# JiahaoPlus/EvoWorld

Measured on AMD Instinct MI355X. Metric: panoramic frames/sec per clip (576x1024x25f, 25 denoise steps), higher is better.
Workload: dtype f16

## Files before the change

evoworld_amd/csrc/norm.hip:

```cpp
#include "common.h"
#include <cstdlib>

namespace {

inline int gn_chunks(int n_slabs, int rows) {
    constexpr int target = 640;
    int want = (target + n_slabs - 1) / n_slabs;
    const int cap = (rows + 63) / 64;
    if (want > cap) want = cap;
    if (want > 512) want = 512;
    return want < 1 ? 1 : want;
}

__device__ __forceinline__ void gn_chan(float& na, float& ma, float& Ma, float nb, float mb, float Mb) {
    if (nb > 0.f) {
        const float n = na + nb, w = __fdividef(nb, n), d = mb - ma;
        ma = fmaf(d, w, ma);
        Ma = fmaf(d * d, na * w, Ma + Mb);
        na = n;
    }
}

__global__ void gn_stats_kernel(const f16* __restrict__ x, const int8_t* __restrict__ x_lo, float* __restrict__ part,
                                int rows, int C_src, int c_off, int C_tot, int VPP, int PL, int rows_per_block) {
    extern __shared__ float lds[];
    const int tid = threadIdx.x;
    const int slab = blockIdx.y;
    const int v = tid % VPP, pl = tid / VPP;
    const int r0 = blockIdx.x * rows_per_block;
    const int r1 = min(rows, r0 + rows_per_block);
    const int nb = max(r1 - r0, 0), nlo = nb / PL, nrem = nb - nlo * PL;
    const int nt = nlo + (pl < nrem ? 1 : 0);
    float s[8], q[8], piv[8];
    const size_t slab_off = ((size_t)slab * rows) * C_src + v * 8;
    const f16* base = x + slab_off;
    const int8_t* base_lo = x_lo ? x_lo + slab_off : nullptr;
#pragma unroll
    for (int e = 0; e < 8; ++e) { s[e] = 0.f; q[e] = 0.f; piv[e] = 0.f; }
    if (nt > 0) {
        const size_t o = (size_t)(r0 + pl) * C_src;
        const f16x8 p0 = *(const f16x8*)(base + o);
#pragma unroll
        for (int e = 0; e < 8; ++e) piv[e] = (float)p0[e];
        if (base_lo) ew_split_dec8(p0, *(const u32x2*)(base_lo + o), piv);
    }
    int r = r0 + pl;
    if (base_lo) {
        constexpr int UL = 8;
        for (; r + (UL - 1) * PL < r1; r += UL * PL) {
            f16x8 val[UL];
            u32x2 vlo[UL];
#pragma unroll
            for (int u = 0; u < UL; ++u) {
                val[u] = *(const f16x8*)(base + (size_t)(r + u * PL) * C_src);
                vlo[u] = *(const u32x2*)(base_lo + (size_t)(r + u * PL) * C_src);
            }
#pragma unroll
            for (int u = 0; u < UL; ++u) {
                float xv[8];
                ew_split_dec8(val[u], vlo[u], xv);
#pragma unroll
                for (int e = 0; e < 8; ++e) {
                    const float f = xv[e] - piv[e];
                    s[e] += f;
                    q[e] += f * f;
                }
            }
        }
        for (; r < r1; r += PL) {
            const f16x8 val = *(const f16x8*)(base + (size_t)r * C_src);
            float xv[8];
            ew_split_dec8(val, *(const u32x2*)(base_lo + (size_t)r * C_src), xv);
#pragma unroll
            for (int e = 0; e < 8; ++e) {
                const float f = xv[e] - piv[e];
                s[e] += f;
                q[e] += f * f;
            }
        }
    } else {
        for (; r + 7 * PL < r1; r += 8 * PL) {
            f16x8 val[8];
#pragma unroll
            for (int u = 0; u < 8; ++u) val[u] = *(const f16x8*)(base + (size_t)(r + u * PL) * C_src);
#pragma unroll
            for (int u = 0; u < 8; ++u)
#pragma unroll
                for (int e = 0; e < 8; ++e) {
                    const float f = (float)val[u][e] - piv[e];
                    s[e] += f;
                    q[e] += f * f;
                }
        }
        for (; r < r1; r += PL) {
            const f16x8 val = *(const f16x8*)(base + (size_t)r * C_src);
#pragma unroll
            for (int e = 0; e < 8; ++e) {
                const float f = (float)val[e] - piv[e];
                s[e] += f;
                q[e] += f * f;
            }
        }
    }
    float* mine = lds + (size_t)pl * 2 * C_src;
    const float inv_n = 1.f / (float)max(nt, 1);
#pragma unroll
    for (int e = 0; e < 8; ++e) {
        const float d = s[e] * inv_n;
        mine[v * 8 + e] = piv[e] + d;
        mine[C_src + v * 8 + e] = fmaxf(q[e] - s[e] * d, 0.f);
    }
    __syncthreads();
    float* dst = part + (((size_t)slab * gridDim.x + blockIdx.x) * C_tot + c_off) * 2;
    for (int c = tid; c < C_src; c += blockDim.x) {
        const float ref = lds[c];
        float sd = 0.f;
        for (int k = 0; k < PL; ++k) sd += (float)(nlo + (k < nrem ? 1 : 0)) * (lds[(size_t)k * 2 * C_src + c] - ref);
        const float dm = nb > 0 ? sd / (float)nb : 0.f;
        float M2 = 0.f;
        for (int k = 0; k < PL; ++k) {
            const float dk = lds[(size_t)k * 2 * C_src + c] - ref - dm;
            M2 += lds[(size_t)k * 2 * C_src + C_src + c] + (float)(nlo + (k < nrem ? 1 : 0)) * dk * dk;
        }
        *(f32x2*)(dst + 2 * c) = (f32x2){ref + dm, M2};
    }
}

__global__ __launch_bounds__(256) void gn_finalize_kernel(const float* __restrict__ part, float* __restrict__ stats, int n_slabs,
                                                          int rows, int C_tot, int groups, int chunks) {
    __shared__ float red[3][256];
    __shared__ float chan[2][512];
    __shared__ float wsum[4];
    const int tid = threadIdx.x;
    const int slab = blockIdx.x / groups, g = blockIdx.x - slab * groups;
    const int gs = C_tot / groups;
    const float n = (float)rows;
    const int cw = gs < 256 ? gs : 256;
    const int KP = 256 / cw;
    const int rpb = (rows + chunks - 1) / chunks;
    for (int c0 = 0; c0 < gs; c0 += cw) {
        const int c = c0 + tid % cw, kc = tid / cw;
        float na = 0.f, ma = 0.f, Ma = 0.f, ref = 0.f;
        if (kc < KP && c < gs) {
            const float* p = part + (((size_t)slab * chunks) * C_tot + g * gs + c) * 2;
            ref = p[0];
            for (int k = kc; k < chunks; k += KP) {
                const f32x2 v = *(const f32x2*)(p + (size_t)k * C_tot * 2);
                gn_chan(na, ma, Ma, (float)max(min(rows - k * rpb, rpb), 0), v[0] - ref, v[1]);
            }
        }
        red[0][tid] = na;
        red[1][tid] = ma;
        red[2][tid] = Ma;
        __syncthreads();
        if (tid < cw && c0 + tid < gs) {
            const int lanes = min(KP, chunks);
            float sd = 0.f, M = 0.f;
            for (int k = 0; k < lanes; ++k) sd += red[0][k * cw + tid] * red[1][k * cw + tid];
            const float dm = sd / n;
            for (int k = 0; k < lanes; ++k) {
                const float dk = red[1][k * cw + tid] - dm;
                M += red[2][k * cw + tid] + red[0][k * cw + tid] * dk * dk;
            }
            chan[0][c0 + tid] = ref + dm;
            chan[1][c0 + tid] = M;
        }
        __syncthreads();
    }
    float ms = 0.f, m2 = 0.f;
    for (int c = tid; c < gs; c += 256) { ms += chan[0][c]; m2 += chan[1][c]; }
    ms = wave_sum(ms);
    m2 = wave_sum(m2);
    if ((tid & 63) == 0) wsum[tid >> 6] = ms;
    __syncthreads();
    const float mean = (wsum[0] + wsum[1] + wsum[2] + wsum[3]) / (float)gs;
    __syncthreads();
    float dev = 0.f;
    for (int c = tid; c < gs; c += 256) { const float d = chan[0][c] - mean; dev += d * d; }
    dev = wave_sum(dev);
    if ((tid & 63) == 0) { wsum[tid >> 6] = m2 + n * dev; }
    __syncthreads();
    if (tid == 0) *(f32x2*)(stats + (size_t)blockIdx.x * 2) = (f32x2){mean, (wsum[0] + wsum[1] + wsum[2] + wsum[3]) / (n * (float)gs)};
}

template <bool LO, bool YLO>
__global__ void gn_apply_kernel(const f16* __restrict__ x, const int8_t* __restrict__ x_lo, const float* __restrict__ stats,
                                const f16* __restrict__ gamma, const f16* __restrict__ beta, f16* __restrict__ y,
                                f16* __restrict__ y_lo, int ld_y, int rows,
                                int C_src, int c_off, int C_tot, int groups, float eps, int silu, int VPP, int PL,
                                int rows_per_block) {
    const int tid = threadIdx.x;
    const int slab = blockIdx.y;
    const int v = tid % VPP, pl = tid / VPP;
    const int c = v * 8;
    const int gs = C_tot / groups;
    const f16x8 gm = *(const f16x8*)(gamma + c_off + c);
    const f16x8 bt = *(const f16x8*)(beta + c_off + c);
    float scale[8], shift[8];
    int gprev = -1;
    float mean = 0.f, rstd = 0.f;
#pragma unroll
    for (int e = 0; e < 8; ++e) {
        const int g = (c_off + c + e) / gs;
        if (g != gprev) {
            gprev = g;
            const f32x2 st = *(const f32x2*)(stats + ((size_t)slab * groups + g) * 2);
            mean = st[0];
            rstd = rsqrtf(st[1] + eps);
        }
        scale[e] = rstd;
        shift[e] = mean;
    }
    const int r0 = blockIdx.x * rows_per_block;
    const int r1 = min(rows, r0 + rows_per_block);
    const f16* xin = x + ((size_t)slab * rows) * C_src + c;
    const int8_t* xlo = LO ? x_lo + ((size_t)slab * rows) * C_src + c : nullptr;
    f16* yout = y + ((size_t)slab * rows) * ld_y + c_off + c;
    f16* ylo = YLO ? y_lo + ((size_t)slab * rows) * ld_y + c_off + c : nullptr;
    int r = r0 + pl;
    for (; r + 3 * PL < r1; r += 4 * PL) {
        f16x8 val[4];
        u32x2 vlo[4];
#pragma unroll
        for (int u = 0; u < 4; ++u) {
            val[u] = *(const f16x8*)(xin + (size_t)(r + u * PL) * C_src);
            if constexpr (LO) vlo[u] = *(const u32x2*)(xlo + (size_t)(r + u * PL) * C_src);
        }
#pragma unroll
        for (int u = 0; u < 4; ++u) {
            f16x8 o, ol;
#pragma unroll
            for (int e = 0; e < 8; ++e) {
                float xv;
                if constexpr (LO) xv = ew_split_dec(val[u][e], ew_sbyte(vlo[u][e >> 2], e & 3));
                else xv = (float)val[u][e];
                float f = (xv - shift[e]) * scale[e] * (float)gm[e] + (float)bt[e];
                if (silu) f = ew_silu(f);
                o[e] = (f16)f;
                if constexpr (YLO) ol[e] = (f16)(f - (float)o[e]);
            }
            *(f16x8*)(yout + (size_t)(r + u * PL) * ld_y) = o;
            if constexpr (YLO) *(f16x8*)(ylo + (size_t)(r + u * PL) * ld_y) = ol;
        }
    }
    for (; r < r1; r += PL) {
        const f16x8 val = *(const f16x8*)(xin + (size_t)r * C_src);
        u32x2 vlo;
        if constexpr (LO) vlo = *(const u32x2*)(xlo + (size_t)r * C_src);
        f16x8 o, ol;
#pragma unroll
        for (int e = 0; e < 8; ++e) {
            float xv;
            if constexpr (LO) xv = ew_split_dec(val[e], ew_sbyte(vlo[e >> 2], e & 3));
            else xv = (float)val[e];
            float f = (xv - shift[e]) * scale[e] * (float)gm[e] + (float)bt[e];
            if (silu) f = ew_silu(f);
            o[e] = (f16)f;
            if constexpr (YLO) ol[e] = (f16)(f - (float)o[e]);
        }
        *(f16x8*)(yout + (size_t)r * ld_y) = o;
        if constexpr (YLO) *(f16x8*)(ylo + (size_t)r * ld_y) = ol;
    }
}

template <int NV, int RPW>
__global__ __launch_bounds__(256) void ln_kernel(const f16* __restrict__ x, const int8_t* __restrict__ x_lo,
                                                 const f16* __restrict__ addvec, int rpg, f16* __restrict__ x_out,
                                                 int8_t* __restrict__ x_out_lo, const f16* __restrict__ gamma,
                                                 const f16* __restrict__ beta, f16* __restrict__ y, int rows, int C,
                                                 float eps) {
    const int lane = threadIdx.x & 63;
    const int row0 = (blockIdx.x * 4 + (threadIdx.x >> 6)) * RPW;
    if (row0 >= rows) return;
    const int VPP = C / 8;
    float v[RPW][NV][8];
    f16x8 raw[RPW][NV], add[RPW][NV];
    u32x2 rlo[RPW][NV];
#pragma unroll
    for (int r = 0; r < RPW; ++r) {
        const int row = min(row0 + r, rows - 1);
#pragma unroll
        for (int k = 0; k < NV; ++k) {
            const int vi = lane + k * 64;
            if (vi < VPP) {
                raw[r][k] = *(const f16x8*)(x + (size_t)row * C + vi * 8);
                if (x_lo) rlo[r][k] = *(const u32x2*)(x_lo + (size_t)row * C + vi * 8);
                if (addvec) add[r][k] = *(const f16x8*)(addvec + (size_t)(row / rpg) * C + vi * 8);
            }
        }
    }
    f16x8 g[NV], bta[NV];
#pragma unroll
    for (int k = 0; k < NV; ++k) {
        const int vi = lane + k * 64;
        if (vi < VPP) { g[k] = *(const f16x8*)(gamma + vi * 8); bta[k] = *(const f16x8*)(beta + vi * 8); }
    }
#pragma unroll
    for (int r = 0; r < RPW; ++r) {
        const int row = row0 + r;
        const bool live = row < rows;
        float sum = 0.f;
#pragma unroll
        for (int k = 0; k < NV; ++k) {
            const int vi = lane + k * 64;
            if (vi < VPP) {
                if (x_lo) {
                    ew_split_dec8(raw[r][k], rlo[r][k], v[r][k]);
                } else {
#pragma unroll
                    for (int e = 0; e < 8; ++e) v[r][k][e] = (float)raw[r][k][e];
                }
                if (addvec) {
                    f16x8 xo;
                    int s8[8];
#pragma unroll
                    for (int e = 0; e < 8; ++e) {
                        const float sum = v[r][k][e] + (float)add[r][k][e];
                        xo[e] = (f16)sum;
                        s8[e] = ew_split_enc(sum, xo[e]);
                        v[r][k][e] = !x_out ? sum : (x_out_lo ? ew_split_dec(xo[e], s8[e]) : (float)xo[e]);
                    }
                    if (x_out && live) *(f16x8*)(x_out + (size_t)row * C + vi * 8) = xo;
                    if (x_out_lo && live)
                        *(u32x2*)(x_out_lo + (size_t)row * C + vi * 8) =
                            (u32x2){ew_pack4(s8[0], s8[1], s8[2], s8[3]), ew_pack4(s8[4], s8[5], s8[6], s8[7])};
                }
#pragma unroll
                for (int e = 0; e < 8; ++e) sum += v[r][k][e];
            } else {
#pragma unroll
                for (int e = 0; e < 8; ++e) v[r][k][e] = 0.f;
            }
        }
        const float mean = wave_sum(sum) / (float)C;
        float sq = 0.f;
#pragma unroll
        for (int k = 0; k < NV; ++k) {
            const int vi = lane + k * 64;
            if (vi < VPP) {
#pragma unroll
                for (int e = 0; e < 8; ++e) { const float d = v[r][k][e] - mean; sq += d * d; }
            }
        }
        const float rstd = rsqrtf(wave_sum(sq) / (float)C + eps);
#pragma unroll
        for (int k = 0; k < NV; ++k) {
            const int vi = lane + k * 64;
            if (vi < VPP && live) {
                f16x8 o;
#pragma unroll
                for (int e = 0; e < 8; ++e) o[e] = (f16)((v[r][k][e] - mean) * rstd * (float)g[k][e] + (float)bta[k][e]);
                *(f16x8*)(y + (size_t)row * C + vi * 8) = o;
            }
        }
    }
}

}

extern "C" size_t ew_groupnorm_workspace_floats(int n_slabs, int rows, int C_tot, int groups) {
    if (n_slabs <= 0 || rows <= 0 || C_tot <= 0 || groups <= 0) return 0;
    return (size_t)n_slabs * gn_chunks(n_slabs, rows) * C_tot * 2 + (size_t)n_slabs * groups * 2;
}

namespace {
struct GnWs { float* part; float* stats; int chunks; };
inline GnWs gn_ws(float* ws, int n_slabs, int rows, int C_tot) {
    GnWs w;
    w.chunks = gn_chunks(n_slabs, rows);
    w.part = ws;
    w.stats = ws + (size_t)n_slabs * w.chunks * C_tot * 2;
    return w;
}
}

extern "C" ew_status ew_groupnorm_stats_f16(const void* x, const void* x_lo, float* ws, int n_slabs, int rows, int C_src,
                                            int c_off, int C_tot, int groups, void* stream) {
    EW_REQUIRE(x && ws, "ew_groupnorm_stats_f16: null pointer");
    EW_REQUIRE(n_slabs > 0 && rows > 0 && C_src > 0 && C_src % 8 == 0 && C_src <= 8192, "ew_groupnorm_stats_f16: bad shape");
    EW_REQUIRE(groups > 0 && C_tot % groups == 0 && c_off >= 0 && c_off + C_src <= C_tot, "ew_groupnorm_stats_f16: bad groups");
    const int VPP = C_src / 8;
    EW_REQUIRE(VPP <= 1024, "ew_groupnorm_stats_f16: C_src too large");
    const int PL = VPP >= 256 ? 1 : 256 / VPP;
    const GnWs w = gn_ws(ws, n_slabs, rows, C_tot);
    const int rpb = ew_cdiv(rows, w.chunks);
    dim3 grid(w.chunks, n_slabs);
    const size_t lds = (size_t)PL * 2 * C_src * sizeof(float);
    EW_REQUIRE(lds <= 64 * 1024, "ew_groupnorm_stats_f16: C_src too large for the LDS combine");
    hipLaunchKernelGGL(gn_stats_kernel, grid, dim3(VPP * PL), lds, (hipStream_t)stream, (const f16*)x, (const int8_t*)x_lo,
                       w.part, rows, C_src, c_off, C_tot, VPP, PL, rpb);
    return ew_check_launch("ew_groupnorm_stats_f16");
}

extern "C" ew_status ew_groupnorm_finalize(float* ws, int n_slabs, int rows, int C_tot, int groups, void* stream) {
    EW_REQUIRE(ws, "ew_groupnorm_finalize: null pointer");
    EW_REQUIRE(n_slabs > 0 && rows > 0 && groups > 0 && C_tot % groups == 0 && C_tot / groups <= 512,
               "ew_groupnorm_finalize: bad shape");
    const GnWs w = gn_ws(ws, n_slabs, rows, C_tot);
    hipLaunchKernelGGL(gn_finalize_kernel, dim3(n_slabs * groups), dim3(256), 0, (hipStream_t)stream,
                       w.part, w.stats, n_slabs, rows, C_tot, groups, w.chunks);
    return ew_check_launch("ew_groupnorm_finalize");
}

static ew_status gn_apply_launch(const char* what, const void* x, const void* x_lo, const float* ws, const void* gamma,
                                 const void* beta, void* y, void* y_lo, int ld_y, int n_slabs, int rows, int C_src, int c_off,
                                 int C_tot, int groups, float eps, int silu, void* stream) {
    EW_REQUIRE(x && ws && gamma && beta && y, "ew_groupnorm_apply: null pointer");
    EW_REQUIRE(n_slabs > 0 && rows > 0 && C_src > 0 && C_src % 8 == 0 && c_off % 8 == 0 && C_tot % 8 == 0,
               "ew_groupnorm_apply: bad shape");
    EW_REQUIRE(groups > 0 && C_tot % groups == 0 && c_off >= 0 && c_off + C_src <= C_tot, "ew_groupnorm_apply: bad groups");
    EW_REQUIRE(ld_y >= C_tot && ld_y % 8 == 0, "ew_groupnorm_apply: bad output row stride");
    const int VPP = C_src / 8;
    EW_REQUIRE(VPP <= 1024, "ew_groupnorm_apply: C_src too large");
    const int PL = VPP >= 256 ? 1 : 256 / VPP;
    const int rpb = 8 * PL;
    const GnWs w = gn_ws((float*)ws, n_slabs, rows, C_tot);
    dim3 grid(ew_cdiv(rows, rpb), n_slabs);
#define GN_APPLY(LO_, YLO_)                                                                                                      \
    hipLaunchKernelGGL((gn_apply_kernel<LO_, YLO_>), grid, dim3(VPP * PL), 0, (hipStream_t)stream, (const f16*)x,                  \
                       (const int8_t*)x_lo, w.stats, (const f16*)gamma, (const f16*)beta, (f16*)y, (f16*)y_lo, ld_y, rows, C_src,  \
                       c_off, C_tot, groups, eps, silu, VPP, PL, rpb)
    if (x_lo) { if (y_lo) GN_APPLY(true, true); else GN_APPLY(true, false); }
    else      { if (y_lo) GN_APPLY(false, true); else GN_APPLY(false, false); }
#undef GN_APPLY
    return ew_check_launch(what);
}

extern "C" ew_status ew_groupnorm_apply_f16(const void* x, const void* x_lo, const float* ws, const void* gamma,
                                            const void* beta, void* y, int n_slabs, int rows, int C_src, int c_off, int C_tot,
                                            int groups, float eps, int silu, void* stream) {
    return gn_apply_launch("ew_groupnorm_apply_f16", x, x_lo, ws, gamma, beta, y, nullptr, C_tot, n_slabs, rows, C_src, c_off, C_tot,
                           groups, eps, silu, stream);
}

extern "C" ew_status ew_groupnorm_apply_split_f16(const void* x, const void* x_lo, const float* ws, const void* gamma,
                                                  const void* beta, void* y, void* y_lo, int ld_y, int n_slabs, int rows, int C_src,
                                                  int c_off, int C_tot, int groups, float eps, int silu, void* stream) {
    EW_REQUIRE(y_lo, "ew_groupnorm_apply_split_f16: null pointer");
    return gn_apply_launch("ew_groupnorm_apply_split_f16", x, x_lo, ws, gamma, beta, y, y_lo, ld_y, n_slabs, rows, C_src, c_off, C_tot,
                           groups, eps, silu, stream);
}

extern "C" ew_status ew_layernorm_f16(const void* x, const void* x_lo, const void* addvec, int rows_per_group, void* x_out,
                                      void* x_out_lo, const void* gamma, const void* beta, void* y, int rows, int C, float eps,
                                      void* stream) {
    EW_REQUIRE(x && gamma && beta && y, "ew_layernorm_f16: null pointer");
    EW_REQUIRE(rows > 0 && C > 0 && C % 8 == 0 && C <= 2048, "ew_layernorm_f16: need C %% 8 == 0 and C <= 2048 (C=%d)", C);
    EW_REQUIRE(!addvec || rows_per_group >= 1, "ew_layernorm_f16: rows_per_group must be >= 1");
    EW_REQUIRE(!x_out_lo || (addvec && x_out), "ew_layernorm_f16: x_out_lo needs addvec and x_out");
    const int nv = (C / 8 + 63) / 64;
    dim3 block(256);
    hipStream_t s = (hipStream_t)stream;
    const int rpg = rows_per_group >= 1 ? rows_per_group : 1;
#define LN_LAUNCH(NV, RPW)                                                                                         \
    hipLaunchKernelGGL((ln_kernel<NV, RPW>), dim3(ew_cdiv(rows, 4 * RPW)), block, 0, s, (const f16*)x, (const int8_t*)x_lo, \
                       (const f16*)addvec, rpg, (f16*)x_out, (int8_t*)x_out_lo, (const f16*)gamma, (const f16*)beta, (f16*)y, rows, C, eps)
    if (nv == 1) LN_LAUNCH(1, 4);
    else if (nv == 2) LN_LAUNCH(2, 4);
    else if (nv == 3) LN_LAUNCH(3, 2);
    else LN_LAUNCH(4, 2);
#undef LN_LAUNCH
    return ew_check_launch("ew_layernorm_f16");
}
```

evoworld_amd/ops.py:

```python
import ctypes

import numpy as np
import torch

from . import _lib
from ._lib import GemmArgs

A_DENSE, A_CONV3X3, A_CONVT3 = _lib.EW_A_DENSE, _lib.EW_A_CONV3X3, _lib.EW_A_CONVT3
ACT_NONE, ACT_SILU, ACT_GEGLU, ACT_GELU = _lib.EW_ACT_NONE, _lib.EW_ACT_SILU, _lib.EW_ACT_GEGLU, _lib.EW_ACT_GELU

_zero_pages = {}


def _stream():
    return ctypes.c_void_p(torch.cuda.current_stream().cuda_stream)


def _ptr(t):
    return None if t is None else ctypes.c_void_p(t.data_ptr())


def _call(name, *args):
    _lib.check(getattr(_lib.load(), name)(*args, _stream()), name)


def _aligned(t, n=16):
    t = t.contiguous()
    return t if t.data_ptr() % n == 0 else t.clone(memory_format=torch.contiguous_format)


def _req(t, dtype, name):
    if t.device.type != "cuda":
        raise _lib.EvoWorldHipError(f"{name} must live on the GPU (got {t.device}); evoworld_amd has no CPU path")
    if t.dtype != dtype:
        raise TypeError(f"{name}: expected {dtype}, got {t.dtype}")
    if not t.is_contiguous():
        raise ValueError(f"{name} must be contiguous")
    return t


def zero_page(device):
    key = str(device)
    if key not in _zero_pages:
        _zero_pages[key] = torch.zeros(4096, dtype=torch.float16, device=device)
    return _zero_pages[key]


class Res:
    __slots__ = ("hi", "lo")

    def __init__(self, hi, lo=None):
        self.hi, self.lo = hi, lo

    @classmethod
    def empty(cls, rows, C, device, split):
        hi = torch.empty(rows, C, dtype=torch.float16, device=device)
        return cls(hi, torch.empty(rows, C, dtype=torch.int8, device=device) if split else None)

    @classmethod
    def from_float(cls, x):
        x = x.float().contiguous()
        hi = x.half()
        d = (x.view(torch.int32) - hi.float().view(torch.int32) + 16) >> 5
        return cls(hi, d.clamp_(-128, 127).to(torch.int8))

    def float(self):
        if self.lo is None:
            return self.hi.float()
        return (self.hi.float().contiguous().view(torch.int32) + (self.lo.to(torch.int32) << 5)).view(torch.float32)


def _hl(x):
    if x is None:
        return None, None
    if isinstance(x, Res):
        return x.hi, x.lo
    return x, None


def gemm(a, w, out, *, M, N, c1, lda, a2=None, c2=0, lda2=0, bias=None, rowbias=None, rows_per_group=1, ld_rowbias=None,
         r1=None, ld_r1=0, r2=None, ld_r2=0, ld_out=None, mode=A_DENSE, conv=None, tconv=None, act=ACT_NONE,
         c_acc=1.0, c_r1=1.0, c_r2=1.0, conv_shift=0):
    g = GemmArgs()
    r1h, r1l = _hl(r1)
    r2h, r2l = _hl(r2)
    outh, outl = _hl(out)
    g.a, g.a2, g.w, g.bias, g.rowbias = _ptr(a), _ptr(a2), _ptr(w), _ptr(bias), _ptr(rowbias)
    g.r1, g.r2, g.out, g.zero_page = _ptr(r1h), _ptr(r2h), _ptr(outh), _ptr(zero_page(a.device))
    g.r1_lo, g.r2_lo, g.out_lo = _ptr(r1l), _ptr(r2l), _ptr(outl)
    g.M, g.N, g.c1, g.c2, g.lda, g.lda2 = M, N, c1, c2, lda, lda2
    n_out = N // 2 if act == ACT_GEGLU else N
    g.ld_out = ld_out if ld_out is not None else n_out
    g.ld_r1, g.ld_r2, g.mode = ld_r1, ld_r2, mode
    g.ld_rowbias = ld_rowbias if ld_rowbias is not None else N
    if conv is not None:
        g.n_img, g.h_in, g.w_in, g.h_out, g.w_out, g.stride, g.upsample = conv
    if tconv is not None:
        g.tB, g.tT, g.tP = tconv
    g.rows_per_group, g.act = rows_per_group, act
    g.c_acc, g.c_r1, g.c_r2 = c_acc, c_r1, c_r2
    g.conv_shift = conv_shift
    _call("ew_gemm_f16", ctypes.byref(g))
    return out


_sk_ready = set()


def streamk_init():
    key = (torch.cuda.current_device(), torch.cuda.current_stream().cuda_stream)
    if key in _sk_ready:
        return
    if _lib.load().ew_get_gemm_generation() != 3:
        return
    if torch.cuda.is_current_stream_capturing():
        return
    _sk_ready.add(key)
    if _lib.load().ew_gemm_streamk_init(_stream()) != 0:
        import warnings
        msg = _lib.load().ew_last_error()
        warnings.warn("ew_gemm_streamk_init: " + (msg.decode() if msg else "failed") + " (continuing without the stream-K tail on this stream)")


def streamk_check():
    st = _lib.load().ew_gemm_streamk_status()
    if st != 0:
        msg = _lib.load().ew_last_error()
        raise _lib.EvoWorldHipError((msg.decode() if msg else "stream-K hand-over timed out in ew_gemm_f16 (generation 3): results of that launch are invalid")
                                    if st > 0 else "ew_gemm_streamk_status: HIP error while reading the status word")


def linear(x, w, bias=None, out=None, split_out=False, **kw):
    _req(x, torch.float16, "x"); _req(w, torch.float16, "w")
    M, K = x.shape
    N = w.shape[0]
    act = kw.get("act", ACT_NONE)
    if out is None:
        n_out = N // 2 if act == ACT_GEGLU else N
        out = Res.empty(M, n_out, x.device, True) if split_out else torch.empty(M, n_out, dtype=torch.float16, device=x.device)
    return gemm(x, w, out, M=M, N=N, c1=K, lda=K, bias=bias, **kw)


class WorkspacePool:

    def __init__(self, device, floats=8 << 20):
        self.buf = torch.empty(floats, dtype=torch.float32, device=device)
        self.cur = 0

    def reset(self):
        self.cur = 0

    def take(self, n):
        n = (n + 63) // 64 * 64
        if self.cur + n > self.buf.numel():
            return torch.empty(n, dtype=torch.float32, device=self.buf.device)
        v = self.buf[self.cur: self.cur + n]
        self.cur += n
        return v


def groupnorm(xs, gamma, beta, n_slabs, rows, eps, silu, groups=32, out=None, pool=None, stats_hi_only=False, split_out=False):
    lib = _lib.load()
    srcs = [_hl(x) for x in xs]
    C_tot = sum(h.shape[-1] for h, _ in srcs)
    dev = srcs[0][0].device
    nws = lib.ew_groupnorm_workspace_floats(n_slabs, rows, C_tot, groups)
    ws = pool.take(nws) if pool is not None else torch.empty(nws, dtype=torch.float32, device=dev)
    if out is None:
        out = torch.empty(n_slabs * rows, 2 * C_tot if split_out else C_tot, dtype=torch.float16, device=dev)
    off = 0
    for h, l in srcs:
        _call("ew_groupnorm_stats_f16", _ptr(h), None if stats_hi_only else _ptr(l), _ptr(ws), n_slabs, rows, h.shape[-1], off, C_tot, groups)
        off += h.shape[-1]
    _call("ew_groupnorm_finalize", _ptr(ws), n_slabs, rows, C_tot, groups)
    off = 0
    for h, l in srcs:
        if split_out:
            _call("ew_groupnorm_apply_split_f16", _ptr(h), _ptr(l), _ptr(ws), _ptr(gamma), _ptr(beta), _ptr(out), _ptr(out[:, C_tot:]),
                  2 * C_tot, n_slabs, rows, h.shape[-1], off, C_tot, groups, eps, 1 if silu else 0)
        else:
            _call("ew_groupnorm_apply_f16", _ptr(h), _ptr(l), _ptr(ws), _ptr(gamma), _ptr(beta), _ptr(out), n_slabs, rows,
                  h.shape[-1], off, C_tot, groups, eps, 1 if silu else 0)
        off += h.shape[-1]
    return out


def layernorm(x, gamma, beta, eps=1e-5, addvec=None, rows_per_group=1, x_out=None, out=None):
    xh, xl = _hl(x)
    oh, ol = _hl(x_out)
    rows, C = xh.shape
    if out is None:
        out = torch.empty_like(xh)
    _call("ew_layernorm_f16", _ptr(xh), _ptr(xl), _ptr(addvec), rows_per_group, _ptr(oh), _ptr(ol), _ptr(gamma), _ptr(beta), _ptr(out), rows, C, eps)
    return out


def attn_spatial(q, k, vt, o, n_seq, S, heads, ld_qk, ld_vt, ld_o, scale=0.125):
    _call("ew_attn_spatial_f16", _ptr(q), _ptr(k), _ptr(vt), _ptr(o), n_seq, S, heads, ld_qk, ld_vt, ld_o, scale)
    return o


QK_LOG2_PRESCALE = (0.125 * 1.4426950408889634) ** 0.5


def attn_spatial_log2(q, k, vt, o, n_seq, S, heads, ld_qk, ld_vt, ld_o):
    _call("ew_attn_spatial_log2_f16", _ptr(q), _ptr(k), _ptr(vt), _ptr(o), n_seq, S, heads, ld_qk, ld_vt, ld_o)
    return o


def quant_rows_fp8(x):
    _req(x, torch.float16, "x")
    if x.ndim != 2:
        raise ValueError(f"x: expected fp16 [rows, K], got {tuple(x.shape)}")
    rows, K = x.shape
    q = torch.empty(rows, K, dtype=torch.uint8, device=x.device)
    scale = torch.empty(rows, dtype=torch.float32, device=x.device)
    _call("ew_quant_rows_fp8", _ptr(x), _ptr(q), _ptr(scale), rows, K)
    return q, scale


def gemm_fp8(aq, a_scale, wq, w_scale, out=None, c_acc=1.0):
    _req(aq, torch.uint8, "aq"); _req(wq, torch.uint8, "wq"); _req(a_scale, torch.float32, "a_scale"); _req(w_scale, torch.float32, "w_scale")
    if aq.ndim != 2 or wq.ndim != 2 or aq.shape[1] != wq.shape[1]:
        raise ValueError(f"aq {tuple(aq.shape)} / wq {tuple(wq.shape)}: expected [M, K] and [N, K]")
    M, K = aq.shape
    N = wq.shape[0]
    if a_scale.numel() != M or w_scale.numel() != N:
        raise ValueError(f"a_scale / w_scale hold {a_scale.numel()} / {w_scale.numel()} values for M, N = {M}, {N}")
    if out is None:
        out = torch.empty(M, N, dtype=torch.float16, device=aq.device)
    if out.dtype != torch.float16 or out.device != aq.device or tuple(out.shape) != (M, N) or out.stride(1) != 1:
        raise ValueError(f"out: expected an fp16 [{M}, {N}] device tensor with unit column stride, got {out.dtype} {tuple(out.shape)} strides {out.stride()}")
    _call("ew_gemm_fp8", _ptr(aq), _ptr(a_scale), _ptr(wq), _ptr(w_scale), _ptr(out), M, N, K, out.stride(0), float(c_acc))
    return out


def attn_temporal(q, k, v, o, B, T, S, heads, ld, ld_o, scale=0.125):
    _call("ew_attn_temporal_f16", _ptr(q), _ptr(k), _ptr(v), _ptr(o), B, T, S, heads, ld, ld_o, scale)
    return o


def softmax_rows(scores, out=None):
    h, l = _hl(scores)
    R, C = h.shape
    if out is None:
        out = torch.empty_like(h)
    _call("ew_softmax_rows_f16", _ptr(h), _ptr(l), _ptr(out), R, C, C)
    return out


def time_conv3(x, w, bias):
    _req(x, torch.float32, "x"); _req(w, torch.float32, "w"); _req(bias, torch.float32, "bias")
    B, T, C, H, W = x.shape
    y = torch.empty_like(x)
    _call("ew_time_conv3_f32", _ptr(x), _ptr(w), _ptr(bias), _ptr(y), B, T, C, H * W)
    return y


def sinusoid_embed(vals, n_rows, dim):
    _req(vals, torch.float32, "vals")
    out = torch.empty(n_rows, dim, dtype=torch.float16, device=vals.device)
    _call("ew_sinusoid_embed_f16", _ptr(vals), vals.numel(), n_rows, dim, _ptr(out))
    return out


def nchw_f32_to_nhwc_f16(x, y, ldc, c_off=0, scale=1.0, split=None):
    _req(x, torch.float32, "x"); _req(y, torch.float16, "y")
    N, C, H, W = x.shape
    if split:
        _call("ew_nchw_f32_to_nhwc_split_f16", _ptr(x), _ptr(y), N, C, H, W, ldc, c_off, split[0], split[1], scale)
        return y
    _call("ew_nchw_f32_to_nhwc_f16", _ptr(x), _ptr(y), N, C, H, W, ldc, c_off, scale)
    return y


def nhwc_f16_to_nchw_f32(x, N, C, H, W, ldc):
    _req(x, torch.float16, "x")
    y = torch.empty(N, C, H, W, dtype=torch.float32, device=x.device)
    _call("ew_nhwc_f16_to_nchw_f32", _ptr(x), _ptr(y), N, C, H, W, ldc)
    return y


def euler_cfg_step(eps, ld_eps, latents, guidance, sigma, sigma_next, next_in, cpad, T, h, w, split=None):
    _req(latents, torch.float32, "latents"); _req(guidance, torch.float32, "guidance")
    if split:
        _call("ew_euler_cfg_step_split", _ptr(eps), ld_eps, _ptr(latents), _ptr(guidance), float(sigma), float(sigma_next),
              _ptr(next_in), cpad, split[0], split[1], T, h, w)
        return
    _call("ew_euler_cfg_step", _ptr(eps), ld_eps, _ptr(latents), _ptr(guidance), float(sigma), float(sigma_next), _ptr(next_in), cpad, T, h, w)


def plucker_embed(rays, c2w):
    _req(rays, torch.float32, "rays"); _req(c2w, torch.float32, "c2w")
    H, W, _ = rays.shape
    N = c2w.shape[0]
    out = torch.empty(N, 6, H, W, dtype=torch.float32, device=rays.device)
    _call("ew_plucker_embed", _ptr(rays), _ptr(c2w), _ptr(out), N, H, W)
    return out


def cube2equi_gather(faces, lut, H, W):
    _req(faces, torch.uint8, "faces"); _req(lut, torch.int16, "lut")
    V, res, ch = faces.shape[0], faces.shape[2], faces.shape[-1]
    pano = torch.empty(V, H, W, 3, dtype=torch.uint8, device=faces.device)
    _call("ew_cube2equi_gather", _ptr(faces), ch, _ptr(lut), _ptr(pano), V, H, W, res)
    return pano


def equi2cube(panos, interpolation=True, out=None):
    _req(panos, torch.uint8, "panos")
    if panos.ndim != 4 or panos.shape[3] != 3:
        raise ValueError(f"panos: expected uint8 [V,H,W,3], got {tuple(panos.shape)}")
    V, H, W, _ = panos.shape
    if out is None:
        out = torch.empty(V, 3 * (W // 4), W, 3, dtype=torch.uint8, device=panos.device)
    _req(out, torch.uint8, "out")
    if tuple(out.shape) != (V, 3 * (W // 4), W, 3):
        raise ValueError(f"out: expected {(V, 3 * (W // 4), W, 3)}, got {tuple(out.shape)}")
    _call("ew_equi2cube_u8", _ptr(panos), _ptr(out), V, H, W, int(bool(interpolation)))
    return out


def cubemap_faces_to_equi(faces, H, W):
    from .reprojection import FACE_ORDER, build_cubemap2equi_lut
    if isinstance(faces, dict):
        unknown = set(faces) - set(FACE_ORDER)
        if unknown or not faces:
            raise ValueError(f"faces: expected keys among {FACE_ORDER}, got {sorted(faces)}")
        first = next(iter(faces.values()))
        for n, f in faces.items():
            if f.ndim != 4 or f.shape[1] != f.shape[2] or f.shape[3] != 3 or f.shape != first.shape:
                raise ValueError(f"faces[{n!r}]: expected square uint8 [V,res,res,3] faces of one size, got {tuple(f.shape)}")
        faces = torch.stack([faces[n] if n in faces else torch.zeros_like(first) for n in FACE_ORDER], dim=1)
    lut = build_cubemap2equi_lut(W, H, faces.shape[2]).to(faces.device)
    return cube2equi_gather(faces.contiguous(), lut, H, W)


def select_kth(x, k):
    lib = _lib.load()
    x = _aligned(x)
    _req(x, torch.float32, "x")
    ws = torch.empty(lib.ew_select_workspace_bytes() // 4 + 4, dtype=torch.int32, device=x.device)
    out = torch.empty(2, dtype=torch.float32, device=x.device)
    _call("ew_select_kth_f32", _ptr(x), x.numel(), int(k), _ptr(ws), _ptr(out))
    return out


def filter_compact(conf, thr, xyz, img, img_nchw_hw=0):
    lib = _lib.load()
    conf, xyz, img = _aligned(conf), _aligned(xyz), _aligned(img)
    _req(conf, torch.float32, "conf"); _req(xyz, torch.float32, "xyz"); _req(img, torch.float32, "img")
    n = conf.numel()
    dev = conf.device
    out_xyz = torch.empty(n, 3, dtype=torch.float32, device=dev)
    out_rgbx = torch.empty(n, 4, dtype=torch.uint8, device=dev)
    ws = torch.empty(lib.ew_filter_compact_workspace_bytes(n) // 4 + 1, dtype=torch.int32, device=dev)
    total = torch.zeros(1, dtype=torch.int32, device=dev)
    _call("ew_filter_compact", _ptr(conf), n, float(thr), _ptr(xyz), _ptr(img), 1 if img_nchw_hw else 0, int(img_nchw_hw),
          _ptr(out_xyz), _ptr(out_rgbx), _ptr(ws), _ptr(total))
    m = int(total.item())
    return out_xyz[:m], out_rgbx[:m]


def depth_unproject(depth, extr, intr):
    _req(depth, torch.float32, "depth"); _req(extr, torch.float32, "extr"); _req(intr, torch.float32, "intr")
    S, H, W = depth.shape
    xyz = torch.empty(S, H, W, 3, dtype=torch.float32, device=depth.device)
    _call("ew_depth_unproject", _ptr(depth), _ptr(extr), _ptr(intr), _ptr(xyz), S, H, W)
    return xyz


def splat_cubemap(xyz, rgb, w2c, res, fx, fy, cx, cy, z_near, face_channels=3):
    xyz = _aligned(xyz)
    _req(xyz, torch.float32, "xyz"); _req(w2c, torch.float32, "w2c")
    if rgb.dtype != torch.uint8 or rgb.device.type != "cuda":
        raise TypeError("rgb must be a uint8 device tensor")
    if rgb.ndim == 2 and rgb.stride(0) == 4 and rgb.stride(1) == 1:
        stride = 4
    else:
        rgb, stride = rgb.contiguous(), 3
    V = w2c.shape[0]
    zbuf = torch.empty((V, 6, res, res), dtype=torch.int64, device=xyz.device)
    _call("ew_splat_cubemap", _ptr(xyz), xyz.shape[0], _ptr(w2c), _ptr(zbuf), V, res, fx, fy, cx, cy, z_near)
    faces = torch.empty(V, 6, res, res, face_channels, dtype=torch.uint8, device=xyz.device)
    _call("ew_splat_resolve", _ptr(zbuf), _ptr(rgb), stride, _ptr(faces), face_channels, V, res)
    return faces, zbuf


def points_bounds(xyz):
    lib = _lib.load()
    xyz = _aligned(xyz)
    _req(xyz, torch.float32, "xyz")
    n = xyz.shape[0]
    if xyz.ndim != 2 or xyz.shape[1] != 3:
        raise ValueError(f"xyz must be [n,3], got {tuple(xyz.shape)}")
    ws = torch.empty(lib.ew_points_bounds_workspace_bytes(n) // 8 + 1, dtype=torch.int64, device=xyz.device)
    out6 = torch.empty(6, dtype=torch.float32, device=xyz.device)
    cnt = torch.empty(1, dtype=torch.int64, device=xyz.device)
    _call("ew_points_bounds", _ptr(xyz), n, _ptr(ws), _ptr(out6), _ptr(cnt))
    b = out6.cpu().numpy()
    return b[:3].copy(), b[3:].copy(), int(cnt.item())


VOXEL_GRID_BITS = 21


def voxel_downsample(xyz, rgbx, voxel_size):
    try:
        v = float(voxel_size)
    except (TypeError, ValueError):
        raise ValueError(f"voxel_size must be a positive finite number, got {voxel_size!r}") from None
    v32 = np.float32(v)
    if not (np.isfinite(v32) and v32 > 0):
        raise ValueError(f"voxel_size must be a positive finite number (in float32), got {voxel_size!r}")
    if rgbx.dtype != torch.uint8 or rgbx.device.type != "cuda":
        raise TypeError("rgbx must be a uint8 device tensor")
    if xyz.ndim != 2 or xyz.shape[1] != 3 or rgbx.ndim != 2 or rgbx.shape[0] != xyz.shape[0] or rgbx.shape[1] not in (3, 4):
        raise ValueError(f"xyz must be [n,3] and rgbx [n,3|4], got {tuple(xyz.shape)} and {tuple(rgbx.shape)}")
    dev = xyz.device

    def empty():
        return (torch.empty(0, 3, dtype=torch.float32, device=dev), torch.empty(0, 4, dtype=torch.uint8, device=dev),
                torch.empty(0, dtype=torch.int32, device=dev))

    n = xyz.shape[0]
    if n == 0:
        return empty()
    lib = _lib.load()
    xyz = _aligned(xyz)
    _req(xyz, torch.float32, "xyz")
    if rgbx.shape[1] == 3:
        rgbx = torch.cat([rgbx, torch.zeros(n, 1, dtype=torch.uint8, device=dev)], dim=1)
    rgbx = _aligned(rgbx)
    lo, hi, n_finite = points_bounds(xyz)
    if n_finite == 0:
        return empty()
    origin = (lo - np.float32(0.5) * v32).astype(np.float32)
    origin_d = torch.from_numpy(origin).to(dev)
    keys = torch.empty(n, dtype=torch.int64, device=dev)
    overflow = torch.zeros(1, dtype=torch.int32, device=dev)
    _call("ew_voxel_keys", _ptr(xyz), n, _ptr(origin_d), float(v32), _ptr(keys), _ptr(overflow))
    if int(overflow.item()):
        extent = float(np.max(hi.astype(np.float64) - lo.astype(np.float64)))
        raise ValueError(f"voxel_size {v:g} is too small for a cloud of extent {extent:g}: a voxel key has {VOXEL_GRID_BITS} bits per "
                         f"axis, so the smallest voxel size this cloud admits is about {extent / 2 ** VOXEL_GRID_BITS:g} "
                         f"(extent / 2^{VOXEL_GRID_BITS})")
    skeys, perm = torch.sort(keys, stable=True)
    out_xyz = torch.empty(n, 3, dtype=torch.float32, device=dev)
    out_rgba = torch.empty(n, 4, dtype=torch.uint8, device=dev)
    out_cnt = torch.empty(n, dtype=torch.int32, device=dev)
    ws = torch.empty(lib.ew_voxel_reduce_workspace_bytes(n) // 16 + 1, 2, dtype=torch.int64, device=dev)
    m_d = torch.empty(1, dtype=torch.int64, device=dev)
    _call("ew_voxel_reduce", _ptr(skeys), _ptr(perm), n, _ptr(xyz), _ptr(rgbx), _ptr(out_xyz), _ptr(out_rgba), _ptr(out_cnt), _ptr(ws),
          _ptr(m_d))
    m = int(m_d.item())
    return out_xyz[:m], out_rgba[:m], out_cnt[:m]


JPEG_SAMPLING = {"4:2:0": (_lib.EW_JPEG_420, 16, 6), "4:4:4": (_lib.EW_JPEG_444, 8, 3)}


def jpeg_dct_quant(frames_u8, quality, subsampling="4:2:0", out=None):
    _req(frames_u8, torch.uint8, "frames_u8")
    if frames_u8.ndim != 4 or frames_u8.shape[3] != 3:
        raise ValueError(f"frames_u8 must be [V,H,W,3], got {tuple(frames_u8.shape)}")
    if subsampling not in JPEG_SAMPLING:
        raise ValueError(f"subsampling must be one of {sorted(JPEG_SAMPLING)}, got {subsampling!r}")
    if not (isinstance(quality, int) and 1 <= quality <= 100):
        raise ValueError(f"quality must be an integer 1..100, got {quality!r}")
    V, H, W, _ = frames_u8.shape
    if not (1 <= V <= 65535 and 1 <= H <= 65535 and 1 <= W <= 65535):
        raise ValueError(f"V, H and W must be 1..65535, got {V}, {H}, {W}")
    mode, mcu, bpm = JPEG_SAMPLING[subsampling]
    shape = (V, -(-H // mcu), -(-W // mcu), bpm, 64)
    if out is None:
        out = torch.empty(shape, dtype=torch.int16, device=frames_u8.device)
    elif tuple(out.shape) != shape:
# ... 674 lines not shown
```

Before: 5.270.

## Pre-reduce GroupNorm statistics per group inside the stats kernel

The stats kernel now folds its per-channel partials into per-group mean/M2 partials in LDS, using 8-lane shuffles. Channels of groups split across concatenated sources keep a per-channel fallback. The finalize kernel shrinks to one 64-thread wave per group that merges only these group partials instead of every channel partial. Finalize is also launched from the apply entry point rather than as a separate Python call, and the chunk cap is raised so each slab is split into more row chunks. The aim is to cut finalize memory traffic and per-call host overhead, at the cost of a longer stats-kernel epilogue and a redundant finalize launch per source when inputs are concatenated.

```diff
diff --git a/evoworld_amd/csrc/norm.hip b/evoworld_amd/csrc/norm.hip
--- a/evoworld_amd/csrc/norm.hip
+++ b/evoworld_amd/csrc/norm.hip
@@ -6,23 +6,21 @@
 inline int gn_chunks(int n_slabs, int rows) {
     constexpr int target = 640;
     int want = (target + n_slabs - 1) / n_slabs;
-    const int cap = (rows + 63) / 64;
+    const int cap = (rows + 15) / 16;
     if (want > cap) want = cap;
     if (want > 512) want = 512;
     return want < 1 ? 1 : want;
 }
 
-__device__ __forceinline__ void gn_chan(float& na, float& ma, float& Ma, float nb, float mb, float Mb) {
-    if (nb > 0.f) {
-        const float n = na + nb, w = __fdividef(nb, n), d = mb - ma;
-        ma = fmaf(d, w, ma);
-        Ma = fmaf(d * d, na * w, Ma + Mb);
-        na = n;
-    }
-}
-
-__global__ void gn_stats_kernel(const f16* __restrict__ x, const int8_t* __restrict__ x_lo, float* __restrict__ part,
-                                int rows, int C_src, int c_off, int C_tot, int VPP, int PL, int rows_per_block) {
+__device__ __forceinline__ float gn_sum8(float v) {
+#pragma unroll
+    for (int o = 4; o > 0; o >>= 1) v += __shfl_xor(v, o, 8);
+    return v;
+}
+
+__global__ void gn_stats_kernel(const f16* __restrict__ x, const int8_t* __restrict__ x_lo, float* __restrict__ gpart,
+                                float* __restrict__ ext, float* __restrict__ cpart, int rows, int C_src, int c_off, int C_tot,
+                                int groups, int VPP, int PL, int rows_per_block) {
     extern __shared__ float lds[];
     const int tid = threadIdx.x;
     const int slab = blockIdx.y;
@@ -111,7 +109,8 @@
         mine[C_src + v * 8 + e] = fmaxf(q[e] - s[e] * d, 0.f);
     }
     __syncthreads();
-    float* dst = part + (((size_t)slab * gridDim.x + blockIdx.x) * C_tot + c_off) * 2;
+    const size_t blk = (size_t)slab * gridDim.x + blockIdx.x;
+    float* cdst = cpart + (blk * C_tot + c_off) * 2;
     for (int c = tid; c < C_src; c += blockDim.x) {
         const float ref = lds[c];
         float sd = 0.f;
@@ -122,65 +121,94 @@
             const float dk = lds[(size_t)k * 2 * C_src + c] - ref - dm;
             M2 += lds[(size_t)k * 2 * C_src + C_src + c] + (float)(nlo + (k < nrem ? 1 : 0)) * dk * dk;
         }
-        *(f32x2*)(dst + 2 * c) = (f32x2){ref + dm, M2};
-    }
-}
-
-__global__ __launch_bounds__(256) void gn_finalize_kernel(const float* __restrict__ part, float* __restrict__ stats, int n_slabs,
-                                                          int rows, int C_tot, int groups, int chunks) {
-    __shared__ float red[3][256];
-    __shared__ float chan[2][512];
-    __shared__ float wsum[4];
-    const int tid = threadIdx.x;
+        lds[c] = ref + dm;
+        lds[C_src + c] = M2;
+        *(f32x2*)(cdst + 2 * c) = (f32x2){ref + dm, M2};
+    }
+    __syncthreads();
+    const int gs = C_tot / groups;
+    const int g_lo = c_off / gs, ng = (c_off + C_src - 1) / gs - g_lo + 1;
+    const int sub = tid & 7;
+    if (tid < (int)(blockDim.x & ~7u)) {
+        for (int i = tid >> 3; i < ng; i += blockDim.x >> 3) {
+            const int g = g_lo + i, g0 = g * gs;
+            const int a = max(g0, c_off) - c_off, b = min(g0 + gs, c_off + C_src) - c_off;
+            const bool head = c_off <= g0, tail = c_off + C_src >= g0 + gs;
+            if (!head && !tail) continue;
+            const float ref = lds[a];
+            float sd = 0.f;
+            for (int c = a + sub; c < b; c += 8) sd += lds[c] - ref;
+            const float dm = gn_sum8(sd) / (float)(b - a);
+            float M2 = 0.f, dev = 0.f;
+            for (int c = a + sub; c < b; c += 8) {
+                const float dc = lds[c] - ref - dm;
+                dev += dc * dc;
+                M2 += lds[C_src + c];
+            }
+            M2 = gn_sum8(M2) + (float)nb * gn_sum8(dev);
+            if (sub == 0) {
+                float* slots = gpart + (blk * groups + g) * 4;
+                if (head) *(f32x2*)slots = (f32x2){ref + dm, M2};
+                if (tail) *(f32x2*)(slots + 2) = head ? (f32x2){0.f, 0.f} : (f32x2){ref + dm, M2};
+                if (blk == 0) {
+                    if (head) ext[g * 2] = (float)(b - a);
+                    if (tail) ext[g * 2 + 1] = head ? 0.f : (float)(b - a);
+                }
+            }
+        }
+    }
+}
+
+template <class F>
+__device__ __forceinline__ void gn_group_items(const float* s0, int sstride, const float* __restrict__ cp, int g, int gs, int C_tot,
+                                               int rows, int crows, int nch0, int nch1, int k0, int kstep, int chunks, F f) {
+    for (int k = k0; k < chunks; k += kstep) {
+        const float nk = (float)max(min(rows - k * crows, crows), 0);
+        const float* s = s0 + (size_t)k * sstride;
+        const f32x2 h = *(const f32x2*)s;
+        f(nk * (float)nch0, h[0], h[1]);
+        if (nch1 > 0) {
+            const f32x2 t = *(const f32x2*)(s + 2);
+            f(nk * (float)nch1, t[0], t[1]);
+        }
+        for (int c = g * gs + nch0; c < (g + 1) * gs - nch1; ++c) {
+            const f32x2 p = *(const f32x2*)(cp + ((size_t)k * C_tot + c) * 2);
+            f(nk, p[0], p[1]);
+        }
+    }
+}
+
+__device__ __forceinline__ void gn_group_extent(const float* __restrict__ ext, int g, int gs, int& nch0, int& nch1) {
+    nch0 = min(max((int)ext[g * 2], 1), gs);
+    nch1 = min(max((int)ext[g * 2 + 1], 0), gs - nch0);
+}
+
+__device__ __forceinline__ f32x2 gn_group_combine(const float* s0, int sstride, const float* __restrict__ cp, int g, int gs, int C_tot,
+                                                  int rows, int crows, int nch0, int nch1, int k0, int kstep, int chunks) {
+    const float ref = s0[0];
+    float sd = 0.f;
+    gn_group_items(s0, sstride, cp, g, gs, C_tot, rows, crows, nch0, nch1, k0, kstep, chunks,
+                   [&](float n, float m, float) { sd += n * (m - ref); });
+    sd = wave_sum(sd);
+    const float N = (float)rows * (float)gs;
+    const float dm = sd / N;
+    float M2 = 0.f;
+    gn_group_items(s0, sstride, cp, g, gs, C_tot, rows, crows, nch0, nch1, k0, kstep, chunks,
+                   [&](float n, float m, float M) { const float d = m - ref - dm; M2 += M + n * d * d; });
+    M2 = wave_sum(M2);
+    return (f32x2){ref + dm, M2 / N};
+}
+
+__global__ __launch_bounds__(64) void gn_finalize_kernel(const float* __restrict__ gpart, const float* __restrict__ ext,
+                                                         const float* __restrict__ cpart, float* __restrict__ stats, int rows,
+                                                         int C_tot, int groups, int chunks, int crows) {
     const int slab = blockIdx.x / groups, g = blockIdx.x - slab * groups;
     const int gs = C_tot / groups;
-    const float n = (float)rows;
-    const int cw = gs < 256 ? gs : 256;
-    const int KP = 256 / cw;
-    const int rpb = (rows + chunks - 1) / chunks;
-    for (int c0 = 0; c0 < gs; c0 += cw) {
-        const int c = c0 + tid % cw, kc = tid / cw;
-        float na = 0.f, ma = 0.f, Ma = 0.f, ref = 0.f;
-        if (kc < KP && c < gs) {
-            const float* p = part + (((size_t)slab * chunks) * C_tot + g * gs + c) * 2;
-            ref = p[0];
-            for (int k = kc; k < chunks; k += KP) {
-                const f32x2 v = *(const f32x2*)(p + (size_t)k * C_tot * 2);
-                gn_chan(na, ma, Ma, (float)max(min(rows - k * rpb, rpb), 0), v[0] - ref, v[1]);
-            }
-        }
-        red[0][tid] = na;
-        red[1][tid] = ma;
-        red[2][tid] = Ma;
-        __syncthreads();
-        if (tid < cw && c0 + tid < gs) {
-            const int lanes = min(KP, chunks);
-            float sd = 0.f, M = 0.f;
-            for (int k = 0; k < lanes; ++k) sd += red[0][k * cw + tid] * red[1][k * cw + tid];
-            const float dm = sd / n;
-            for (int k = 0; k < lanes; ++k) {
-                const float dk = red[1][k * cw + tid] - dm;
-                M += red[2][k * cw + tid] + red[0][k * cw + tid] * dk * dk;
-            }
-            chan[0][c0 + tid] = ref + dm;
-            chan[1][c0 + tid] = M;
-        }
-        __syncthreads();
-    }
-    float ms = 0.f, m2 = 0.f;
-    for (int c = tid; c < gs; c += 256) { ms += chan[0][c]; m2 += chan[1][c]; }
-    ms = wave_sum(ms);
-    m2 = wave_sum(m2);
-    if ((tid & 63) == 0) wsum[tid >> 6] = ms;
-    __syncthreads();
-    const float mean = (wsum[0] + wsum[1] + wsum[2] + wsum[3]) / (float)gs;
-    __syncthreads();
-    float dev = 0.f;
-    for (int c = tid; c < gs; c += 256) { const float d = chan[0][c] - mean; dev += d * d; }
-    dev = wave_sum(dev);
-    if ((tid & 63) == 0) { wsum[tid >> 6] = m2 + n * dev; }
-    __syncthreads();
-    if (tid == 0) *(f32x2*)(stats + (size_t)blockIdx.x * 2) = (f32x2){mean, (wsum[0] + wsum[1] + wsum[2] + wsum[3]) / (n * (float)gs)};
+    int nch0, nch1;
+    gn_group_extent(ext, g, gs, nch0, nch1);
+    const f32x2 st = gn_group_combine(gpart + ((size_t)slab * chunks * groups + g) * 4, groups * 4, cpart + (size_t)slab * chunks * C_tot * 2,
+                                            g, gs, C_tot, rows, crows, nch0, nch1, threadIdx.x, 64, chunks);
+    if (threadIdx.x == 0) *(f32x2*)(stats + (size_t)blockIdx.x * 2) = st;
 }
 
 template <bool LO, bool YLO>
@@ -360,17 +388,25 @@
 
 extern "C" size_t ew_groupnorm_workspace_floats(int n_slabs, int rows, int C_tot, int groups) {
     if (n_slabs <= 0 || rows <= 0 || C_tot <= 0 || groups <= 0) return 0;
-    return (size_t)n_slabs * gn_chunks(n_slabs, rows) * C_tot * 2 + (size_t)n_slabs * groups * 2;
+    const size_t blocks = (size_t)n_slabs * gn_chunks(n_slabs, rows);
+    return blocks * groups * 4 + (size_t)groups * 2 + blocks * C_tot * 2 + (size_t)n_slabs * groups * 2;
 }
 
 namespace {
-struct GnWs { float* part; float* stats; int chunks; };
-inline GnWs gn_ws(float* ws, int n_slabs, int rows, int C_tot) {
+struct GnWs { float* gpart; float* ext; float* cpart; float* stats; int chunks; };
+inline GnWs gn_ws(float* ws, int n_slabs, int rows, int C_tot, int groups) {
     GnWs w;
     w.chunks = gn_chunks(n_slabs, rows);
-    w.part = ws;
-    w.stats = ws + (size_t)n_slabs * w.chunks * C_tot * 2;
+    const size_t blocks = (size_t)n_slabs * w.chunks;
+    w.gpart = ws;
+    w.ext = w.gpart + blocks * groups * 4;
+    w.cpart = w.ext + (size_t)groups * 2;
+    w.stats = w.cpart + blocks * C_tot * 2;
     return w;
+}
+inline void gn_finalize_launch(const GnWs& w, int n_slabs, int rows, int C_tot, int groups, void* stream) {
+    hipLaunchKernelGGL(gn_finalize_kernel, dim3(n_slabs * groups), dim3(64), 0, (hipStream_t)stream, w.gpart, w.ext, w.cpart, w.stats,
+                       rows, C_tot, groups, w.chunks, ew_cdiv(rows, w.chunks));
 }
 }
 
@@ -382,13 +418,13 @@
     const int VPP = C_src / 8;
     EW_REQUIRE(VPP <= 1024, "ew_groupnorm_stats_f16: C_src too large");
     const int PL = VPP >= 256 ? 1 : 256 / VPP;
-    const GnWs w = gn_ws(ws, n_slabs, rows, C_tot);
+    const GnWs w = gn_ws(ws, n_slabs, rows, C_tot, groups);
     const int rpb = ew_cdiv(rows, w.chunks);
     dim3 grid(w.chunks, n_slabs);
     const size_t lds = (size_t)PL * 2 * C_src * sizeof(float);
     EW_REQUIRE(lds <= 64 * 1024, "ew_groupnorm_stats_f16: C_src too large for the LDS combine");
     hipLaunchKernelGGL(gn_stats_kernel, grid, dim3(VPP * PL), lds, (hipStream_t)stream, (const f16*)x, (const int8_t*)x_lo,
-                       w.part, rows, C_src, c_off, C_tot, VPP, PL, rpb);
+                       w.gpart, w.ext, w.cpart, rows, C_src, c_off, C_tot, groups, VPP, PL, rpb);
     return ew_check_launch("ew_groupnorm_stats_f16");
 }
 
@@ -396,9 +432,7 @@
     EW_REQUIRE(ws, "ew_groupnorm_finalize: null pointer");
     EW_REQUIRE(n_slabs > 0 && rows > 0 && groups > 0 && C_tot % groups == 0 && C_tot / groups <= 512,
                "ew_groupnorm_finalize: bad shape");
-    const GnWs w = gn_ws(ws, n_slabs, rows, C_tot);
-    hipLaunchKernelGGL(gn_finalize_kernel, dim3(n_slabs * groups), dim3(256), 0, (hipStream_t)stream,
-                       w.part, w.stats, n_slabs, rows, C_tot, groups, w.chunks);
+    gn_finalize_launch(gn_ws(ws, n_slabs, rows, C_tot, groups), n_slabs, rows, C_tot, groups, stream);
     return ew_check_launch("ew_groupnorm_finalize");
 }
 
@@ -414,7 +448,8 @@
     EW_REQUIRE(VPP <= 1024, "ew_groupnorm_apply: C_src too large");
     const int PL = VPP >= 256 ? 1 : 256 / VPP;
     const int rpb = 8 * PL;
-    const GnWs w = gn_ws((float*)ws, n_slabs, rows, C_tot);
+    const GnWs w = gn_ws((float*)ws, n_slabs, rows, C_tot, groups);
+    gn_finalize_launch(w, n_slabs, rows, C_tot, groups, stream);
     dim3 grid(ew_cdiv(rows, rpb), n_slabs);
 #define GN_APPLY(LO_, YLO_)                                                                                                      \
     hipLaunchKernelGGL((gn_apply_kernel<LO_, YLO_>), grid, dim3(VPP * PL), 0, (hipStream_t)stream, (const f16*)x,                  \
diff --git a/evoworld_amd/ops.py b/evoworld_amd/ops.py
--- a/evoworld_amd/ops.py
+++ b/evoworld_amd/ops.py
@@ -172,7 +172,6 @@
     for h, l in srcs:
         _call("ew_groupnorm_stats_f16", _ptr(h), None if stats_hi_only else _ptr(l), _ptr(ws), n_slabs, rows, h.shape[-1], off, C_tot, groups)
         off += h.shape[-1]
-    _call("ew_groupnorm_finalize", _ptr(ws), n_slabs, rows, C_tot, groups)
     off = 0
     for h, l in srcs:
         if split_out:
```

Measured after the change: 5.287 (median of 6 runs). About the same (+0.3%).
